# SilverlightningY/dmmt-jpeg-encoder

Hardware: AMD Instinct MI355X
Metric: Mpixel/s encoded (4K PPM, q=90) (higher is better)
Workload: dtype f32; 1 GPU; 3840x2160 synthetic RGB u8, 4:4:4, IJG quality 90, 1 frame(s) per step per GPU, pixels in HBM -> JPEG files in HBM, inputs rotating over 12 distinct slots (285 MiB: streamed from HBM); width=3840, height=2160, subsampling=P444, quality=90, parallelism=independent frames x1, lanes=4, input_slots=12

## Files before the change

### dmmt-jpeg-encoder_amd/csrc/entropy.hip

```cpp
#include <hip/hip_runtime.h>
#include <stdint.h>

#include "device_common.hpp"
#include "jpeg_common.hpp"
#include "kernels.hpp"
#include "slot_copy.hpp"

namespace dmmt {

#ifdef DMMT_PHASE_TRACE
static __device__ unsigned long long g_trace[64];
#endif

static_assert(kChunkBlocks == 256 || kChunkBlocks == 512, "one thread per block, one workgroup per chunk");
constexpr int kEmitThreads = kChunkBlocks;
constexpr int kEmitWaves = kEmitThreads / 64;
#ifndef DMMT_EMIT_OCC
#define DMMT_EMIT_OCC 7
#endif
constexpr int kEmitOcc = kChunkBlocks == 256 ? DMMT_EMIT_OCC : 3;

constexpr int kEmitWords = 4 * kChunkBlocks;
constexpr int kStuffPass = 4096;
#ifndef DMMT_EMIT_BRANCHFREE
#define DMMT_EMIT_BRANCHFREE 1
#endif
#ifndef DMMT_TAIL_DMA
#define DMMT_TAIL_DMA 1
#endif
#ifndef DMMT_TAIL_NSEG1
#define DMMT_TAIL_NSEG1 1
#endif
#ifndef DMMT_EMIT_PRIO_ALWAYS
#define DMMT_EMIT_PRIO_ALWAYS 0
#endif
#ifndef DMMT_EMIT_PRIO
#define DMMT_EMIT_PRIO 1
#endif

struct ChunkSpan {
    long long el0;
    int nb;
    int seg;
    bool seg_first, seg_last;
};

__device__ __forceinline__ ChunkSpan chunk_span(const Geom& g, int c) {
    ChunkSpan r;
    r.seg = min(c / g.cps, g.nseg - 1);
    const int j = c - r.seg * g.cps;
    const long long sb = (long long)r.seg * g.seg_blocks;
    const long long se = min(sb + g.seg_blocks, g.bpf);
    r.el0 = sb + (long long)j * kChunkBlocks;
    r.nb = (int)min((long long)kChunkBlocks, se - r.el0);
    r.seg_first = j == 0;
    r.seg_last = r.el0 + r.nb == se;
    return r;
}

__device__ __forceinline__ bool joined_tail(const Geom& g, int c) {
    return c == g.nch - 1 && g.more_after && g.restart_interval == 0;
}

__device__ __forceinline__ int mod_small(int x, int d, uint32_t inv16) {
    return x - (int)__umul24((uint32_t)d, __umul24((uint32_t)x, inv16) >> 16);
}

struct BlockCoef {
    uint32_t w[32];
};

__device__ __forceinline__ void load_block(const int16_t* __restrict__ p, BlockCoef& b) {
    const uint4* q = reinterpret_cast<const uint4*>(p);
#pragma unroll
    for (int i = 0; i < 8; ++i) {
        const uint4 v = q[i];
        b.w[4 * i] = v.x;
        b.w[4 * i + 1] = v.y;
        b.w[4 * i + 2] = v.z;
        b.w[4 * i + 3] = v.w;
    }
}

__device__ __forceinline__ int coef_at(const BlockCoef& b, int k) {
    return (k & 1) ? ((int)b.w[k >> 1] >> 16) : (int)(int16_t)(b.w[k >> 1] & 0xFFFFu);
}

__device__ __forceinline__ void zigzag_in_registers(BlockCoef& b) {
    uint32_t z[32];
#pragma unroll
    for (int j = 0; j < 32; ++j) {
        const int i0 = coef_pos(2 * j), i1 = coef_pos(2 * j + 1);
        const uint32_t lo = (b.w[i0 >> 1] >> (16 * (i0 & 1))) & 0xFFFFu;
        const uint32_t hi = (b.w[i1 >> 1] >> (16 * (i1 & 1))) & 0xFFFFu;
        z[j] = lo | (hi << 16);
    }
#pragma unroll
    for (int j = 0; j < 32; ++j) b.w[j] = z[j];
}

template <typename Sink>
__device__ __forceinline__ void walk_block(const BlockCoef& b, int dcd, const uint2* __restrict__ dctab,
                                           const uint2* __restrict__ actab, Sink& sink, int kmax = 63) {
    {
        const int cat = category_of(dcd);
        const uint2 e = dctab[cat];
        sink(e.x | extra_bits(dcd, cat), (int)e.y);
    }
    const uint2 z = actab[0xF0];
    int l16 = 16;
#pragma unroll
    for (int k = 1; k < 64; ++k) {
        if (k > kmax) continue;
        const int v = coef_at(b, k);
        if (v != 0) {
            const int r16 = 16 * k - l16;
            for (int r = r16 >> 8; r > 0; --r) sink(z.x, (int)z.y);
            const int cat = category_fast(v);
            const uint2 e = actab[(r16 & 0xF0) | cat];
            sink(e.x | extra_bits(v, cat), (int)e.y);
            l16 = 16 * k + 16;
        }
    }
    if (l16 < 16 * 64 || kmax < 63) {
        const uint2 e = actab[0];
        sink(e.x, (int)e.y);
    }
}

struct CountSink {
    uint32_t n = 0;
    __device__ __forceinline__ void operator()(uint32_t, int len) { n += (uint32_t)len; }
};

struct WindowSink {
    uint32_t* img;
    int lo, n;
    unsigned long long acc;
    int nacc;
    int w;
    bool first;
    __device__ __forceinline__ void put(uint32_t word, bool shared) {
        const int i = w - lo;
        if ((unsigned)i < (unsigned)n) {
            if (shared)
                atomicOr(&img[i], word);
            else
                img[i] = word;
        }
    }
    __device__ __forceinline__ void operator()(uint32_t val, int len) {
        acc = (acc << len) | val;
        nacc += len;
        if (nacc >= 32) {
            nacc -= 32;
            put((uint32_t)(acc >> nacc), first);
            first = false;
            ++w;
        }
    }
    __device__ __forceinline__ void finish() {
        if (nacc > 0) put((uint32_t)(acc << (32 - nacc)), true);
    }
};


struct SlotSink {
    uint32_t* slot;
    unsigned long long acc;
    int nacc;
    int wi;
#if DMMT_EMIT_BRANCHFREE
    __device__ __forceinline__ void operator()(uint32_t val, int len) {
        acc = (acc << len) | val;
        nacc += len;
        const int full = nacc >> 5;
        nacc &= 31;
        slot[min(wi, kSlotWords - 1) * kEmitThreads] = (uint32_t)(acc >> nacc);
        wi += full;
    }
#else
    __device__ __forceinline__ void operator()(uint32_t val, int len) {
        acc = (acc << len) | val;
        nacc += len;
        if (nacc >= 32) {
            nacc -= 32;
            slot[min(wi, kSlotWords - 1) * kEmitThreads] = (uint32_t)(acc >> nacc);
            ++wi;
        }
    }
#endif
    __device__ __forceinline__ uint32_t finish() {
        if (nacc > 0 && wi < kSlotWords) slot[wi * kEmitThreads] = (uint32_t)(acc << (32 - nacc));
        return (uint32_t)wi * 32u + (uint32_t)nacc;
    }
};


__device__ __forceinline__ uint32_t bits16_at(uint32_t a, uint32_t b, int p) {
    const unsigned long long x = ((unsigned long long)a << 32) | b;
    return (uint32_t)(x >> (48 - (p & 31))) & 0xFFFFu;
}

struct NoMark {
    template <typename I>
    __device__ void operator()(I) const {}
};
template <typename Mark = NoMark>
__device__ __forceinline__ void fused_offsets(const uint32_t* __restrict__ cbits, const uint32_t* __restrict__ cff,
                              const unsigned long long* __restrict__ cff8, uint8_t* sFF8,
                              const uint32_t* __restrict__ cedge, const Geom& g, unsigned long long* __restrict__ bit0,
                              unsigned long long* __restrict__ outo, unsigned long long* __restrict__ total,
                              unsigned long long* sWaveV, int* sWaveF, Mark mark = Mark());
static_assert(kArriveWords == kArriveFrameWords, "the host sizes the counters");

__global__ __launch_bounds__(kEmitThreads, kEmitOcc) void k_emit(const int16_t* coef, const int16_t* __restrict__ dcdiff,
                                              const uint8_t* __restrict__ lastnz,
                                              const uint32_t* __restrict__ code_tab, Geom g,
                                              uint32_t* __restrict__ stage, uint32_t* __restrict__ chunk_bits,
                                              uint32_t* __restrict__ chunk_ff, uint32_t* __restrict__ chunk_edge,
                                              uint32_t* __restrict__ ac_hist, uint32_t* __restrict__ dc_hist,
                                              int fuse, uint32_t* __restrict__ arrive,
                                              unsigned long long* __restrict__ chunk_bit0,
                                              unsigned long long* __restrict__ chunk_out,
                                              unsigned long long* __restrict__ total_out,
                                              unsigned long long* __restrict__ chunk_ff8, int prio) {
    __shared__ uint2 sTab[2 * 256 + 2 * 16];
    __shared__ uint32_t sW[kEmitWords + 2];
    __shared__ __attribute__((aligned(16))) uint32_t sSlot[kSlotWords * kEmitThreads];
    __shared__ uint32_t sWave[kEmitWaves];
    __shared__ uint32_t sFF[8];
    __shared__ uint32_t sEdge[3];
    __shared__ uint32_t sBin[65];
    __shared__ unsigned long long sOffV[kEmitWaves + 1];
    __shared__ int sOffF[kEmitWaves];
    __shared__ uint32_t sLast;
    using OrderT = std::conditional_t<(kEmitThreads > 256), uint16_t, uint8_t>;
    uint32_t* const sBits = sW;
    OrderT* const sOrder = reinterpret_cast<OrderT*>(sW + kEmitThreads);
    uint8_t* const sKey = reinterpret_cast<uint8_t*>(sW + kEmitThreads + kEmitThreads * (int)sizeof(OrderT) / 4);
    DMMT_TRACE_START;
    const int tid = threadIdx.x, lane = lane_id(), wave = tid >> 6;
    const int frame = blockIdx.y;
    const unsigned chunk = blockIdx.x;
    const ChunkSpan span = chunk_span(g, (int)chunk);
    const long long el0 = span.el0;
    const int nb = span.nb;
    const long long e = (long long)frame * g.bpf + el0 + tid;
    const size_t cid = (size_t)frame * g.nch + chunk;
    const int r0 = (int)((uint32_t)el0 % (uint32_t)g.bpm);
    const uint32_t inv16 = (65536u + (uint32_t)g.bpm - 1u) / (uint32_t)g.bpm;
    const bool valid = tid < nb;
    const uint32_t* ct = code_tab + (size_t)frame * 1024;
    const int tt = tid & 255;
    const uint32_t tac0 = ct[256 + tt], tac1 = ct[768 + tt];
    const uint32_t tdc = ct[((tt & 31) < 16 ? 0 : 512 - 16) + (tt & 31)];
    const uint32_t lz = lastnz[valid ? e : (long long)frame * g.bpf + el0];
    if (tid < 256) {
        const int c = tid & 15;
        sTab[tid] = make_uint2((tac0 & 0xFFFFu) << c, (tac0 >> 16) + c);
        sTab[256 + tid] = make_uint2((tac1 & 0xFFFFu) << c, (tac1 >> 16) + c);
    }
    if (tid < 32) sTab[512 + tid] = make_uint2((tdc & 0xFFFFu) << (tid & 15), (tdc >> 16) + (tid & 15));
    if (chunk == 0) {
        for (int i = tid; i < kHistReps * 512; i += kEmitThreads) ac_hist[(size_t)frame * kHistReps * 512 + i] = 0u;
        for (int i = tid; i < kHistReps * 32; i += kEmitThreads) dc_hist[(size_t)frame * kHistReps * 32 + i] = 0u;
    }
    if (tid < 8) sFF[tid] = 0u;
    if (tid < 3) sEdge[tid] = 0u;
    if (tid < 65) sBin[tid] = 0u;
    const int key = valid ? (int)lz : 64;
    __syncthreads();
    const uint32_t rank = atomicAdd(&sBin[key], 1u);
    __syncthreads();
// ... 442 lines not shown
        bool f = false;
        unsigned long long v = 0;
#pragma unroll
        for (int i = 0; i < KP; ++i)
            if (c0 + i < c1) seg_combine(f, v, first[i], nbits[i] + (c0 + i == 0 ? (uint32_t)g.bit_phase : 0u));
        unsigned long long run = block_segscan_1024(f, v, sWave, sWaveF);
        unsigned long long b0[KP], ob[KP], mine = 0;
#pragma unroll
        for (int i = 0; i < KP; ++i) {
            const int c = c0 + i;
            b0[i] = ob[i] = 0;
            if (c >= c1) continue;
            if (first[i]) run = c == 0 ? (unsigned long long)g.bit_phase : 0ull;
            b0[i] = run;
            const unsigned long long e = run + nbits[i];
            unsigned long long o = ((e + 7) >> 3) - ((run + 7) >> 3);
            const int rsd = (8 - (int)(run & 7)) & 7;
            uint32_t ffc = 0;
#pragma unroll
            for (int r = 0; r < 8; ++r) ffc = r == rsd ? ffr[i][r] : ffc;
            o += ffc;
            if ((e & 7) && (e & ~7ull) >= run) {
                const uint32_t byte = boundary_byte((int)(e & 7), edge[i] & 0xFFFFu, hasn[i], nnext[i], enext[i] >> 16);
                o += byte == 0xFFu ? 1u : 0u;
            }
            if (segl[i] && (c != nch - 1 || (g.more_after && g.restart_interval > 0))) o += 2;
            ob[i] = o;
            mine += o;
            run = e;
        }
        unsigned long long tot = 0;
        unsigned long long orun = block_scan_1024(mine, sWave, &tot);
#pragma unroll
        for (int i = 0; i < KP; ++i) {
            const int c = c0 + i;
            if (c >= c1) continue;
            bit0[c] = b0[i];
            outo[c] = orun;
            orun += ob[i];
        }
        if (tid == 0) total_out[frame] = tot;
        return;
    }

    bool f = false;
    unsigned long long v = 0;
    for (int c = c0; c < c1; ++c)
        seg_combine(f, v, chunk_span(g, c).seg_first, cbits[c] + (c == 0 ? (unsigned long long)g.bit_phase : 0ull));
    unsigned long long run = block_segscan_1024(f, v, sWave, sWaveF);
    unsigned long long mine = 0;
    for (int c = c0; c < c1; ++c) {
        if (chunk_span(g, c).seg_first) run = c == 0 ? (unsigned long long)g.bit_phase : 0ull;
        bit0[c] = run;
        mine += chunk_out_bytes(cff, cbits, cedge, g, c, run);
        run += cbits[c];
    }
    unsigned long long tot = 0;
    unsigned long long orun = block_scan_1024(mine, sWave, &tot);
    for (int c = c0; c < c1; ++c) {
        outo[c] = orun;
        orun += chunk_out_bytes(cff, cbits, cedge, g, c, bit0[c]);
    }
    if (tid == 0) total_out[frame] = tot;
}

__global__ __launch_bounds__(256, 8) void k_stuffwrite(const uint32_t* __restrict__ stage,
                                                    const uint32_t* __restrict__ chunk_bits,
                                                    const uint32_t* __restrict__ chunk_edge,
                                                    const unsigned long long* __restrict__ chunk_bit0,
                                                    const unsigned long long* __restrict__ chunk_out,
                                                    const unsigned long long* __restrict__ total_out,
                                                    const uint32_t* __restrict__ hdr_len, Geom g,
                                                    uint8_t* __restrict__ out, size_t out_stride,
                                                    uint32_t* __restrict__ out_len, int* __restrict__ status) {
    __shared__ uint32_t sWave[4];
    __shared__ __attribute__((aligned(16))) uint8_t sOut[2 * kStuffPass + 16];
    const int tid = threadIdx.x, lane = lane_id(), wave = tid >> 6;
    const int frame = blockIdx.y;
    const int c = blockIdx.x;
    const size_t cid = (size_t)frame * g.nch + c;
    const bool last = c == g.nch - 1;
    const size_t cidn = last ? cid : cid + 1;
    const uint32_t hdr = hdr_len[frame];
    const unsigned long long tot = total_out[frame];
    const unsigned long long b0 = chunk_bit0[cid];
    const uint32_t n = chunk_bits[cid], edge = chunk_edge[cid];
    const uint32_t n_next = chunk_bits[cidn], edge_next = chunk_edge[cidn];
    const unsigned long long cout = chunk_out[cid], cout_next = chunk_out[cidn];
    const uint32_t* slot = stage + cid * (size_t)kChunkWordsCap;
    uint32_t wv0[5];
    {
        const uint4 q = *reinterpret_cast<const uint4*>(slot + 4 * tid);
        wv0[0] = q.x, wv0[1] = q.y, wv0[2] = q.z, wv0[3] = q.w;
        wv0[4] = slot[4 * tid + 4];
    }
    asm volatile("" ::"s"(hdr), "s"(tot), "s"(b0), "s"(n), "s"(edge), "s"(n_next), "s"(edge_next), "s"(cout),
                 "s"(cout_next), "v"(wv0[0]), "v"(wv0[1]), "v"(wv0[2]), "v"(wv0[3]), "v"(wv0[4]));
    const unsigned long long end = (unsigned long long)hdr + tot;
    if (end + 2 > out_stride) {
        if (c == 0 && tid == 0) {
            out_len[frame] = 0;
            raise_status(status, 16);
        }
        return;
    }
    {
        const unsigned long long cend = last ? tot : cout_next;
        const unsigned long long sbytes = ((unsigned long long)n + 7) / 8 + 1;
        if (n > (uint32_t)kChunkWordsCap * 32u || cout > cend || cend > tot ||
            (unsigned long long)hdr + cout + 2 * sbytes > out_stride) {
            if (tid == 0) {
                out_len[frame] = 0;
                raise_status(status, 16);
            }
            return;
        }
    }
    const ChunkSpan sp = chunk_span(g, c);
    uint8_t* const base = out + (size_t)frame * out_stride + hdr;
    if (tid == 0) {
        if (last && !g.more_after) {
            base[tot] = 0xFF;
            base[tot + 1] = 0xD9;
            out_len[frame] = (uint32_t)(end + 2);
        } else if (sp.seg_last && g.restart_interval > 0) {
            const unsigned long long at = (last ? tot : cout_next) - 2;
            base[at] = 0xFF;
            base[at + 1] = (uint8_t)(0xD0 + ((g.seg_base + sp.seg) & 7));
            if (last) out_len[frame] = (uint32_t)end;
        } else if (last) {
            out_len[frame] = (uint32_t)end;
        }
    }
    const unsigned long long e = b0 + n;
    const unsigned long long kbeg = (b0 + 7) >> 3, kend = (e + 7) >> 3;
    if (kend <= kbeg) return;
    const unsigned long long nbytes = kend - kbeg;
    const bool shared_tail = (e & 7) != 0;
    uint32_t tail = 0;
    if (shared_tail) {
        const bool jt = joined_tail(g, c);
        const bool has_next = !sp.seg_last || jt;
        tail = boundary_byte((int)(e & 7), edge & 0xFFFFu, has_next,
                             jt ? (uint32_t)g.next_bits : (has_next ? n_next : 0u),
                             jt ? g.next16 : (has_next ? edge_next >> 16 : 0u));
    }
    const unsigned off = (unsigned)(8 * kbeg - b0);
    uint8_t* o = base + cout;
    for (unsigned long long pos = 0; pos < nbytes; pos += kStuffPass) {
        const uint32_t delta = (uint32_t)(reinterpret_cast<uintptr_t>(o) & 15u);
        const unsigned long long kb = pos + 16u * (unsigned)tid;
        const int nvalid = kb < nbytes ? (int)min(16ull, nbytes - kb) : 0;
        uint32_t x[4] = {0u, 0u, 0u, 0u};
        uint32_t cnt = 0;
        if (nvalid) {
            const unsigned long long p = off + 8 * kb;
            const size_t wi = (size_t)(p >> 5);
            const int sh = (int)(p & 31);
            uint32_t wv[5];
#pragma unroll
            for (int i = 0; i < 5; ++i) wv[i] = pos ? slot[wi + i] : wv0[i];
#pragma unroll
            for (int i = 0; i < 4; ++i) x[i] = sh ? (wv[i] << sh) | (wv[i + 1] >> (32 - sh)) : wv[i];
            if (shared_tail && nbytes - 1 - kb < 16) {
                const int j = (int)(nbytes - 1 - kb), sft = 24 - 8 * (j & 3);
                x[j >> 2] = (x[j >> 2] & ~(0xFFu << sft)) | (tail << sft);
            }
#pragma unroll
            for (int i = 0; i < 4; ++i) {
                const int nv = min(max(nvalid - 4 * i, 0), 4);
                const uint32_t vmask = nv ? 0x80808080u & (0xFFFFFFFFu << (32 - 8 * nv)) : 0u;
                const uint32_t t = ~x[i];
                const uint32_t nonzero = (((t & 0x7F7F7F7Fu) + 0x7F7F7F7Fu) | t) & 0x80808080u;
                cnt += (uint32_t)__popc(~nonzero & vmask);
            }
        }
        const uint32_t incl = wave_incl_scan_full_u32(cnt);
        if (lane == 63) sWave[wave] = incl;
        __syncthreads();
        uint32_t pre = incl - cnt;
        for (int q = 0; q < wave; ++q) pre += sWave[q];
        const uint32_t ffs = sWave[0] + sWave[1] + sWave[2] + sWave[3];
        if (nvalid) {
            uint32_t dst = delta + (uint32_t)tid * 16u + pre;
#pragma unroll
            for (int j = 0; j < 16; ++j) {
                if (j < nvalid) {
                    const uint32_t b = (x[j >> 2] >> (24 - 8 * (j & 3))) & 0xFFu;
                    sOut[dst++] = (uint8_t)b;
                    if (b == 0xFFu) sOut[dst++] = 0x00;
                }
            }
        }
        __syncthreads();
        const unsigned long long in_pass = nbytes - pos < (unsigned long long)kStuffPass ? nbytes - pos : kStuffPass;
        const uint32_t len = (uint32_t)in_pass + ffs;
        const uint32_t send = delta + len;
        uint8_t* const oa = o - delta;
        for (uint32_t sb = 16u * (uint32_t)tid; sb < send; sb += 16u * 256u) {
            if (sb >= delta && sb + 16u <= send) {
                *reinterpret_cast<uint4*>(oa + sb) = *reinterpret_cast<const uint4*>(sOut + sb);
            } else {
                for (uint32_t i = max(sb, delta); i < min(sb + 16u, send); ++i) oa[i] = sOut[i];
            }
        }
        o += len;
        __syncthreads();
    }
}

bool offsets_fusable(const Geom& g) { return g.nch <= kFusedOffsetsMaxChunks; }

hipError_t launch_emit(int n_frames, const Geom& g, const Work& w, bool fuse_offsets, hipStream_t st, bool prio) {
    const int fuse = fuse_offsets && offsets_fusable(g) ? 1 : 0;
    hipLaunchKernelGGL(k_emit, dim3(g.nch, n_frames), dim3(kEmitThreads), 0, st, (const int16_t*)w.coef,
                       (const int16_t*)w.dcdiff, (const uint8_t*)w.lastnz, (const uint32_t*)w.code_tab, g, w.stage, w.chunk_bits, w.chunk_ff,
                       w.chunk_edge, w.ac_hist, w.dc_hist, fuse, w.arrive, w.chunk_bit0, w.chunk_out, w.total_out,
                       w.chunk_ff8, prio || DMMT_EMIT_PRIO_ALWAYS ? 1 : 0);
    return hipGetLastError();
}

hipError_t launch_offsets(int n_frames, const Geom& g, const Work& w, hipStream_t st) {
    hipLaunchKernelGGL(k_offsets, dim3(n_frames), dim3(1024), 0, st, (const uint32_t*)w.chunk_bits,
                       (const uint32_t*)w.chunk_ff, (const uint32_t*)w.chunk_edge, g, w.chunk_bit0, w.chunk_out,
                       w.total_out);
    return hipGetLastError();
}

hipError_t launch_stuffwrite(int n_frames, const Geom& g, const Work& w, uint8_t* out, size_t out_stride,
                             uint32_t* out_len, hipStream_t st) {
    hipLaunchKernelGGL(k_stuffwrite, dim3(g.nch, n_frames), dim3(256), 0, st, (const uint32_t*)w.stage,
                       (const uint32_t*)w.chunk_bits, (const uint32_t*)w.chunk_edge,
                       (const unsigned long long*)w.chunk_bit0, (const unsigned long long*)w.chunk_out,
                       (const unsigned long long*)w.total_out, (const uint32_t*)w.hdr_len, g, out, out_stride,
                       out_len, w.status);
    return hipGetLastError();
}

}

#ifdef DMMT_PHASE_TRACE
extern "C" int dmmt_debug_trace_entropy(unsigned long long* out64) {
    if (hipMemcpyFromSymbol(out64, HIP_SYMBOL(dmmt::g_trace), 64 * 8) != hipSuccess) return -1;
    unsigned long long z[64] = {0};
    return hipMemcpyToSymbol(HIP_SYMBOL(dmmt::g_trace), z, sizeof z) == hipSuccess ? 0 : -1;
}
#endif
```

### dmmt-jpeg-encoder_amd/csrc/kernels.hip

```cpp

#include <hip/hip_runtime.h>
#include <stdint.h>
#include <stdlib.h>

#include <type_traits>

#include "dct_quant.hpp"
#include "device_common.hpp"
#include "front_launch.hpp"
#include "jpeg_common.hpp"
#include "kernels.hpp"
#include "surface_load.hpp"
#include "wave_merge.hpp"

namespace dmmt {

#ifdef DMMT_PHASE_TRACE
static __device__ unsigned long long g_trace[64];
#endif

__constant__ uint8_t c_zigzag[64] = {0,  1,  8,  16, 9,  2,  3,  10, 17, 24, 32, 25, 18, 11, 4,  5,
                                     12, 19, 26, 33, 40, 48, 41, 34, 27, 20, 13, 6,  7,  14, 21, 28,
                                     35, 42, 49, 56, 57, 50, 43, 36, 29, 22, 15, 23, 30, 37, 44, 51,
                                     58, 59, 52, 45, 38, 31, 39, 46, 53, 60, 61, 54, 47, 55, 62, 63};
__constant__ uint8_t c_inv_zigzag[64] = {0,  1,  5,  6,  14, 15, 27, 28, 2,  4,  7,  13, 16, 26, 29, 42,
                                         3,  8,  12, 17, 25, 30, 41, 43, 9,  11, 18, 24, 31, 40, 44, 53,
                                         10, 19, 23, 32, 39, 45, 52, 54, 20, 22, 33, 38, 46, 51, 55, 60,
                                         21, 34, 37, 47, 50, 56, 59, 61, 35, 36, 48, 49, 57, 58, 62, 63};

__device__ __forceinline__ void rgb_to_ycbcr(float r, float g, float b, float& y, float& cb, float& cr) {
    const float k128 = 128.0f / 255.0f;
    y = (((r * 0.299f + g * 0.587f) + b * 0.114f) - k128) * 255.0f;
    cb = ((r * -0.1687f + g * -0.3312f) + b * 0.5f) * 255.0f;
    cr = ((r * 0.5f + g * -0.4186f) + b * -0.0813f) * 255.0f;
}


template <typename Sample, int ROWS>
struct RawTile {
    static constexpr int RB = 256 * 3 * (int)sizeof(Sample);
    static constexpr int RC = RB / 16 + 1;
    static constexpr int RS = RC * 16;
    static constexpr int NCHUNK = ROWS * RC;
    static constexpr int NQ = (NCHUNK + 255) / 256;
    static constexpr int BYTES = NCHUNK * 16;

    __device__ static __forceinline__ long long row_start(const Geom& g, int x0, int py) {
        return ((long long)py * g.width + x0) * 3 * (long long)sizeof(Sample);
    }
    __device__ static __forceinline__ int misalign(const uint8_t* fbase, long long start) {
        return (int)(((uintptr_t)fbase + (uintptr_t)start) & 15u);
    }

    __device__ static __forceinline__ int misalign32(const uint8_t* fbase, const Geom& g, int x0, int py) {
        return (int)(((uint32_t)(uintptr_t)fbase + (uint32_t)(py * g.width + x0) * (uint32_t)(3 * sizeof(Sample))) & 15u);
    }

    __device__ static __forceinline__ void load(const uint8_t* __restrict__ fbase, long long fbytes, const Geom& g,
                                                int x0, int y0, int tid, uint4 (&v)[NQ]) {
        const long long last = row_start(g, x0, y0 + ROWS - 1);
        if (x0 + 256 <= g.width && y0 + ROWS <= g.height && row_start(g, x0, y0) >= 16 && last + RB + 16 <= fbytes) {
            const uint8_t* tb = fbase + row_start(g, x0, y0);
            const uint32_t rowpitch = (uint32_t)g.width * (uint32_t)(3 * sizeof(Sample));
#pragma unroll
            for (int i = 0; i < NQ; ++i) {
                const int q = tid + 256 * i;
                const int row = q / RC, j = q - (q / RC) * RC;
                const uint8_t* r = tb + (size_t)((uint32_t)row * rowpitch);
                const uint8_t* a = r - ((uint32_t)(uintptr_t)r & 15u) + 16u * (uint32_t)j;
                v[i] = q < NCHUNK ? ld16_nt(a) : make_uint4(0u, 0u, 0u, 0u);
            }
            return;
        }
        const long long rowbytes = (long long)min(256, g.width - x0) * 3 * (long long)sizeof(Sample);
#pragma unroll
        for (int i = 0; i < NQ; ++i) {
            v[i] = make_uint4(0u, 0u, 0u, 0u);
            const int q = tid + 256 * i;
            const int row = q / RC, j = q - (q / RC) * RC;
            const int py = y0 + row;
            if (q >= NCHUNK || py >= g.height) continue;
            const long long start = row_start(g, x0, py);
            const long long c = start - misalign(fbase, start) + 16LL * j;
            if (c >= start + rowbytes) continue;
            if (c >= 0 && c + 16 <= fbytes) {
                v[i] = ld16_nt(fbase + c);
            } else {
                uint32_t w[4] = {0u, 0u, 0u, 0u};
                for (int k = 0; k < 16; ++k)
                    if (c + k >= 0 && c + k < fbytes) w[k >> 2] |= (uint32_t)fbase[c + k] << (8 * (k & 3));
                v[i] = make_uint4(w[0], w[1], w[2], w[3]);
            }
            const long long keep = start + rowbytes - c;
            if (keep < 16) {
                uint32_t w[4] = {v[i].x, v[i].y, v[i].z, v[i].w};
#pragma unroll
                for (int k = 0; k < 4; ++k) {
                    const long long n = keep - 4 * k;
                    w[k] &= n >= 4 ? 0xFFFFFFFFu : (n <= 0 ? 0u : (1u << (8 * n)) - 1u);
                }
                v[i] = make_uint4(w[0], w[1], w[2], w[3]);
            }
        }
    }

    __device__ static __forceinline__ void stage(uint8_t* sRaw, int tid, const uint4 (&v)[NQ]) {
#pragma unroll
        for (int i = 0; i < NQ; ++i) {
            const int q = tid + 256 * i;
            if (q < NCHUNK) reinterpret_cast<uint4*>(sRaw)[q] = v[i];
        }
    }
};

enum { LAY_TIGHT = 0, LAY_RGB = 1, LAY_RGBX = 2, LAY_PLANAR = 3 };
template <int LAY>
struct SurfLayout {
    static constexpr int NPL = LAY == LAY_PLANAR ? 3 : 1;
    static constexpr int SPP = LAY == LAY_RGBX ? 4 : (LAY == LAY_PLANAR ? 1 : 3);
};
struct SurfMem {
    const uint8_t* base;
    __device__ __forceinline__ void load16(long long off, uint32_t (&w)[4]) const {
        const uint4 v = ld16_nt(base + off);
        w[0] = v.x, w[1] = v.y, w[2] = v.z, w[3] = v.w;
    }
    __device__ __forceinline__ uint32_t load1(long long off) const { return base[off]; }
};
template <typename Sample, int ROWS, int LAY>
struct SurfTile {
    static constexpr int NPL = SurfLayout<LAY>::NPL;
    static constexpr int BPP = SurfLayout<LAY>::SPP * (int)sizeof(Sample);
    static constexpr int RB = 256 * BPP;
    static constexpr int RC = RB / 16 + 1;
    static constexpr int RS = RC * 16;
    static constexpr int NCHUNK = ROWS * NPL * RC;
    static constexpr int NQ = (NCHUNK + 255) / 256;
    static constexpr int BYTES = NCHUNK * 16;

    struct Planes {
        const uint8_t *p0, *p1, *p2;
    };
    __device__ static __forceinline__ Planes planes(const SurfArgs& sa, size_t foff) {
        return Planes{sa.plane[0] + foff, sa.plane[NPL == 1 ? 0 : 1] + foff, sa.plane[NPL == 1 ? 0 : 2] + foff};
    }
    __device__ static __forceinline__ const uint8_t* plane(const Planes& pl, int p) {
        return NPL == 1 || p == 0 ? pl.p0 : (p == 1 ? pl.p1 : pl.p2);
    }
    __device__ static __forceinline__ int misalign32(const uint8_t* pbase, const SurfArgs& sa, int x0, int py) {
        return surf_misalign32((uint32_t)(uintptr_t)pbase, (uint32_t)sa.pitch, BPP, x0, py);
    }

    __device__ static __forceinline__ void load(const SurfArgs& sa, size_t foff, const Geom& g, int x0, int y0, int tid,
                                                uint4 (&v)[NQ]) {
        const Planes pl = planes(sa, foff);
        const long long first = surf_row_start(sa.pitch, BPP, x0, y0);
        if (x0 + 256 <= g.width && y0 + ROWS <= g.height &&
            surf_interior(first, surf_row_start(sa.pitch, BPP, x0, y0 + ROWS - 1), RB, sa.span)) {
#pragma unroll
            for (int i = 0; i < NQ; ++i) {
                const int q = tid + 256 * i;
                const int tr = q / RC, j = q - (q / RC) * RC;
                const int row = tr / NPL, p = tr - (tr / NPL) * NPL;
                const uint8_t* pb = plane(pl, p);
                const long long c = surf_interior_chunk((uint32_t)(uintptr_t)pb, first + (long long)row * sa.pitch, j);
                v[i] = q < NCHUNK ? ld16_nt(pb + c) : make_uint4(0u, 0u, 0u, 0u);
            }
            return;
        }
        const long long rowbytes = surf_row_bytes(g.width, BPP, x0);
#pragma unroll
        for (int i = 0; i < NQ; ++i) {
            v[i] = make_uint4(0u, 0u, 0u, 0u);
            const int q = tid + 256 * i;
            const int tr = q / RC, j = q - (q / RC) * RC;
            const int row = tr / NPL, p = tr - (tr / NPL) * NPL;
            const int py = y0 + row;
            if (q >= NCHUNK || py >= g.height) continue;
            const SurfMem m{plane(pl, p)};
            uint32_t w[4];
            surf_load_chunk(m, surf_row_start(sa.pitch, BPP, x0, py), misalign32(m.base, sa, x0, py), rowbytes, sa.span,
                            j, w);
            v[i] = make_uint4(w[0], w[1], w[2], w[3]);
        }
    }

    __device__ static __forceinline__ void stage(uint8_t* sRaw, int tid, const uint4 (&v)[NQ]) {
// ... 25 lines not shown
    constexpr int SB = (int)sizeof(Sample);
    constexpr int NPL = SurfLayout<LAY>::NPL;
    constexpr int SPP = SurfLayout<LAY>::SPP;
    constexpr int PXB = 8 * SPP * SB;
    constexpr int PXW = PXB / 4;
    constexpr int NCJ = NB * 8;
    constexpr int JPT = (NCJ + 255) / 256;
    using Raw = std::conditional_t<LAY == LAY_TIGHT, RawTile<Sample, ROWS>, SurfTile<Sample, ROWS, LAY>>;

    __shared__ __attribute__((aligned(16))) float sT[NB * BS + 4];
    __shared__ __attribute__((aligned(16))) uint8_t sRaw[Raw::BYTES];
    __shared__ float sLut[256];
    __shared__ float sQ[128];
    __shared__ float sRQ[128];

    DMMT_TRACE_START;
    const int tid = threadIdx.x;
    const int frame = blockIdx.y;
    const uint8_t* fbase = nullptr;
    long long fbytes = 0;
    size_t foff = 0;
    if constexpr (LAY == LAY_TIGHT) {
        fbase = reinterpret_cast<const uint8_t*>(rgb + (size_t)frame * frame_stride);
        fbytes = (long long)g.width * g.height * 3 * SB;
    } else {
        foff = (size_t)frame * frame_stride;
    }
    if (tid < 128) sQ[tid] = qtab[tid];
    if (tid < 128) sRQ[tid] = SB == 4 ? 1.0f / qtab[tid] : c_arai_scale[(tid >> 3) & 7] * (1.0f / qtab[tid]);
    if (SB == 1) sLut[tid] = norm_lut[tid];
    const int col = tid & 7;

    const int tiles_per_row = (g.mcux + TM - 1) / TM;
    const int ntiles = tiles_per_row * g.mcuy;
    int bad = 0;
    const bool check_range = SB != 4 && g.maxval < (SB == 1 ? 255 : 65535);

    uint4 raw[Raw::NQ];
    auto load_tile = [&](int tx0, int ty0) {
        if constexpr (LAY == LAY_TIGHT)
            Raw::load(fbase, fbytes, g, tx0, ty0, tid, raw);
        else
            Raw::load(sa, foff, g, tx0, ty0, tid, raw);
    };
    if ((int)blockIdx.x < ntiles) {
        const int my = blockIdx.x / tiles_per_row;
        load_tile((blockIdx.x - my * tiles_per_row) * TM * 8 * HR, my * ROWS);
    }
    for (int tile = blockIdx.x; tile < ntiles; tile += gridDim.x) {
        const int my = tile / tiles_per_row;
        const int mx0 = (tile - my * tiles_per_row) * TM;
        const int x0 = mx0 * 8 * HR;
        const int y0 = my * ROWS;

        Raw::stage(sRaw, tid, raw);
        __syncthreads();
        {
            const int nt = tile + gridDim.x;
            if (nt < ntiles) {
                const int ny = nt / tiles_per_row;
                load_tile((nt - ny * tiles_per_row) * TM * 8 * HR, ny * ROWS);
            }
        }

        auto phase_a = [&](auto range_check) {
            constexpr bool CHECK = decltype(range_check)::value;
            const int h = tid % SP, job = tid / SP;
            const int c = job % CB, r = job / CB;
            const int lx0 = c * 8 * HR + 8 * h;
            uint32_t pw[VR * NPL][SB == 4 ? 1 : PXW];
            const float* fsrc[VR * NPL];
#pragma unroll
            for (int dy = 0; dy < VR; ++dy) {
#pragma unroll
                for (int p = 0; p < NPL; ++p) {
                    const int ly = r * VR + dy;
                    int mis;
                    if constexpr (LAY == LAY_TIGHT)
                        mis = Raw::misalign32(fbase, g, x0, y0 + ly);
                    else
                        mis = Raw::misalign32(sa.plane[p] + foff, sa, x0, y0 + ly);
                    const uint8_t* src = sRaw + (ly * NPL + p) * Raw::RS + mis + lx0 * SPP * SB;
                    fsrc[dy * NPL + p] = reinterpret_cast<const float*>(src);
                    if constexpr (SB == 4) {
                        pw[dy * NPL + p][0] = 0u;
                    } else if ((mis & 7) == 0) {
#pragma unroll
                        for (int k = 0; k < PXW / 2; ++k) {
                            const uint2 u = reinterpret_cast<const uint2*>(src)[k];
                            pw[dy * NPL + p][2 * k] = u.x;
                            pw[dy * NPL + p][2 * k + 1] = u.y;
                        }
                    } else {
#pragma unroll
                        for (int k = 0; k < PXW; ++k)
                            pw[dy * NPL + p][k] = (uint32_t)src[4 * k] | ((uint32_t)src[4 * k + 1] << 8) |
                                                  ((uint32_t)src[4 * k + 2] << 16) | ((uint32_t)src[4 * k + 3] << 24);
                    }
                }
            }
            float yv[VR][8];
            float cbv[8], crv[8];
            uint32_t smax = 0;
#pragma unroll
            for (int k = 0; k < NCS; ++k) {
                float cbs = 0.0f, crs = 0.0f;
#pragma unroll
                for (int dx = 0; dx < HR; ++dx) {
#pragma unroll
                    for (int dy = 0; dy < VR; ++dy) {
                        const int jx = k * HR + dx;
                        float rr, gg, bb;
                        if constexpr (SB == 4) {
                            if constexpr (LAY == LAY_PLANAR) {
                                rr = fsrc[dy * NPL][jx];
                                gg = fsrc[dy * NPL + 1][jx];
                                bb = fsrc[dy * NPL + 2][jx];
                            } else {
                                rr = fsrc[dy][jx * SPP];
                                gg = fsrc[dy][jx * SPP + 1];
                                bb = fsrc[dy][jx * SPP + 2];
                                if constexpr (LAY != LAY_TIGHT) {
                                    const float s0 = rr;
                                    rr = sa.bgr ? bb : rr;
                                    bb = sa.bgr ? s0 : bb;
                                }
                            }
                        } else {
                            uint32_t sv[3];
#pragma unroll
                            for (int ch = 0; ch < 3; ++ch) {
                                const int si = LAY == LAY_PLANAR ? jx : jx * SPP + ch;
                                const uint32_t* rw = pw[LAY == LAY_PLANAR ? dy * NPL + ch : dy];
                                sv[ch] = SB == 1 ? (rw[si >> 2] >> (8 * (si & 3))) & 0xFFu
                                                 : (rw[si >> 1] >> (16 * (si & 1))) & 0xFFFFu;
                            }
                            if constexpr (LAY == LAY_RGB || LAY == LAY_RGBX) {
                                const uint32_t s0 = sv[0];
                                sv[0] = sa.bgr ? sv[2] : sv[0];
                                sv[2] = sa.bgr ? s0 : sv[2];
                            }
                            if constexpr (CHECK) smax = max(smax, max(sv[0], max(sv[1], sv[2])));
                            if (SB == 1) {
                                rr = sLut[sv[0]];
                                gg = sLut[sv[1]];
                                bb = sLut[sv[2]];
                            } else {
                                rr = norm_lut[sv[0]];
                                gg = norm_lut[sv[1]];
                                bb = norm_lut[sv[2]];
                            }
                        }
                        float y, cb, cr;
                        rgb_to_ycbcr(rr, gg, bb, y, cb, cr);
                        yv[dy][jx] = y;
                        if (dx == 0 && dy == 0) {
                            cbs = cb;
                            crs = cr;
                        } else {
                            cbs = cbs + cb;
                            crs = crs + cr;
                        }
                    }
                }
                if (HR * VR > 1) {
                    cbs = cbs / (float)(HR * VR);
                    crs = crs / (float)(HR * VR);
                }
                cbv[k] = cbs;
                crv[k] = crs;
            }
            if constexpr (CHECK) bad |= (int)(smax > (uint32_t)g.maxval);
#pragma unroll
            for (int dy = 0; dy < VR; ++dy) {
                const int ly = r * VR + dy;
                arai8(yv[dy]);
                float4* o = reinterpret_cast<float4*>(sT + blk_base((ly >> 3) * 32 + c * HR + h) + (ly & 7) * 8);
                o[0] = make_float4(yv[dy][0], yv[dy][1], yv[dy][2], yv[dy][3]);
                o[1] = make_float4(yv[dy][4], yv[dy][5], yv[dy][6], yv[dy][7]);
            }
            if constexpr (SP == 1) {
                arai8(cbv);
                arai8(crv);
                float4* ob = reinterpret_cast<float4*>(sT + blk_base(NYB + c) + r * 8);
                ob[0] = make_float4(cbv[0], cbv[1], cbv[2], cbv[3]);
                ob[1] = make_float4(cbv[4], cbv[5], cbv[6], cbv[7]);
                float4* orr = reinterpret_cast<float4*>(sT + blk_base(NYB + CB + c) + r * 8);
                orr[0] = make_float4(crv[0], crv[1], crv[2], crv[3]);
                orr[1] = make_float4(crv[4], crv[5], crv[6], crv[7]);
            } else {
                float fr[8];
#pragma unroll
                for (int k = 0; k < 4; ++k) {
                    const float send = h ? cbv[k] : crv[k];
                    const float recv = __int_as_float(
                        __builtin_amdgcn_update_dpp(0, __float_as_int(send), 0xB1, 0xF, 0xF, false));
                    fr[k] = h ? recv : cbv[k];
                    fr[4 + k] = h ? crv[k] : recv;
                }
                arai8(fr);
                float4* oc = reinterpret_cast<float4*>(sT + blk_base(NYB + (h ? CB : 0) + c) + r * 8);
                oc[0] = make_float4(fr[0], fr[1], fr[2], fr[3]);
                oc[1] = make_float4(fr[4], fr[5], fr[6], fr[7]);
            }
        };
        if (tid < NJ) {
            if (check_range)
                phase_a(std::integral_constant<bool, true>{});
            else
                phase_a(std::integral_constant<bool, false>{});
        }
        __syncthreads();
        DMMT_TRACE(0);

        const int nvalid = min(TM, g.mcux - mx0) * BPM;
        const long long e0 = (long long)frame * g.bpf + ((long long)my * g.mcux + mx0) * BPM;
        int16_t* const cbase = coef + e0 * 64;
        static_assert(NCJ % 256 == 0, "JPT column jobs for every thread");
#pragma unroll
        for (int jj = 0; jj < JPT; ++jj) {
            const int blk = (tid + 256 * jj) >> 3;
            int x[8];
            {
                const float* q = sQ + (blk < NYB ? 0 : 64) + col;
                const float* rq = sRQ + (blk < NYB ? 0 : 64) + col;
                float v[8];
                const float* tb = sT + blk_base(blk) + col;
#pragma unroll
                for (int i = 0; i < 8; ++i) v[i] = tb[i * 8];
                if constexpr (SB == 4) {
                    arai8(v);
                    quantize_col8(v, q, rq, x);
                } else {
                    arai8_unscaled(v);
                    quantize_col8_scaled(v, q, rq, g.maxval == 0, x);
                }
            }
            int el;
            if (blk < NYB) {
                const int by = blk / 32, bx = blk % 32;
                el = (bx / HR) * BPM + by * HR + (bx % HR);
            } else if (blk < NYB + CB) {
                el = (blk - NYB) * BPM + NLUMA;
            } else {
                el = (blk - NYB - CB) * BPM + NLUMA + 1;
            }
            const bool valid = el < nvalid;
            if (valid) {
                uint32_t pk[4];
#pragma unroll
                for (int i = 0; i < 4; ++i) pk[i] = __builtin_amdgcn_perm((uint32_t)x[2 * i + 1], (uint32_t)x[2 * i], 0x05040100u);
                *reinterpret_cast<uint4*>(cbase + (el * 64 + 8 * col)) = make_uint4(pk[0], pk[1], pk[2], pk[3]);
            }
        }
        DMMT_TRACE(2);
    }

    if (bad) raise_status(status, bad);
    DMMT_TRACE(5);
    DMMT_TRACE_FLUSH(0, 0);
}

template <int HR, int VR, typename Sample, int WPE>
__global__ __launch_bounds__(256, WPE) void k_front(const Sample* __restrict__ rgb, size_t frame_stride, Geom g,
                                               const float* __restrict__ norm_lut,
                                               const float* __restrict__ qtab,
                                               int16_t* __restrict__ coef, int* __restrict__ status) {
    front_body<HR, VR, Sample, LAY_TIGHT>(rgb, frame_stride, SurfArgs{}, g, norm_lut, qtab, coef, status);
}

template <int HR, int VR, typename Sample, int LAY, int WPE>
__global__ __launch_bounds__(256, WPE) void k_front_surf(SurfArgs sa, size_t frame_stride, Geom g,
                                                    const float* __restrict__ norm_lut,
                                                    const float* __restrict__ qtab, int16_t* __restrict__ coef,
                                                    int* __restrict__ status) {
    front_body<HR, VR, Sample, LAY>(nullptr, frame_stride, sa, g, norm_lut, qtab, coef, status);
}

struct HistCoef {
    uint32_t w[32];
};

constexpr int kTailSmallWords = 4 + 4 * 16;
__device__ __forceinline__ void tables_tail(uint8_t* lds, const uint32_t* ac_hist, const uint32_t* dc_hist, int frame,
                                            const Geom& g, uint32_t* __restrict__ code_tab, uint8_t* __restrict__ out,
                                            size_t out_stride, uint32_t* __restrict__ hdr_len,
                                            const uint8_t* __restrict__ qtab_u8, int bits_per_channel,
                                            int* __restrict__ status, int* sCnt, int* sBits);
constexpr int kHistCopies = 4, kHistCopyWords = 545;
constexpr int kTailLdsBytes = 7072;

template <bool CHECK, bool FUSE>
__global__ __launch_bounds__(256) __attribute__((amdgpu_waves_per_eu(8, 8))) void k_hist(const int16_t* __restrict__ coef, int16_t* __restrict__ dcdiff,
                                              uint8_t* __restrict__ lastnz, Geom g,
                                              uint32_t* __restrict__ ac_hist ,
                                              uint32_t* __restrict__ dc_hist ,
                                              int* __restrict__ status, uint32_t* __restrict__ arrive,
                                              uint32_t* __restrict__ code_tab, uint8_t* __restrict__ out,
                                              size_t out_stride, uint32_t* __restrict__ hdr_len,
                                              const uint8_t* __restrict__ qtab_u8, int bits_per_channel) {
    constexpr int NC = kHistCopies, HS = kHistCopyWords;
    constexpr int kWords = FUSE && kTailLdsBytes / 4 > NC * HS ? kTailLdsBytes / 4 : NC * HS;
    __shared__ __attribute__((aligned(16))) uint32_t sH[kWords];
    __shared__ int sSmall[FUSE ? kTailSmallWords : 1];
    __shared__ uint32_t sLastWg;
    const int tid = threadIdx.x;
    const int frame = blockIdx.y;
// ... 904 lines not shown
```

Measured before the change: 191,500 Mpixel/s.

## Restructure AC walk, branch-free byte stuffing, simplified copy-out, FMA color convert

The AC Huffman walk now tests nonzero coefficients directly on packed words in groups of four and exits early past kmax. It also guards the ZRL run loop with a wave-uniform ballot so most waves skip it. Byte stuffing scatters bytes to positions derived from popcounts of the 0xFF mask and writes the zero bytes in a separate sparse loop, replacing the serial per-byte loop. The copy-out loop handles only full 16-byte vectors, with edge bytes written by 32 dedicated threads, and the color conversion uses explicit FMAs for the 0.5 terms when SB!=4, which can change rounding.

Measured after the change: 194,300 Mpixel/s, median of 6. 1.5% higher.

```diff
diff --git a/dmmt-jpeg-encoder_amd/csrc/entropy.hip b/dmmt-jpeg-encoder_amd/csrc/entropy.hip
--- a/dmmt-jpeg-encoder_amd/csrc/entropy.hip
+++ b/dmmt-jpeg-encoder_amd/csrc/entropy.hip
@@ -108,18 +108,29 @@
         sink(e.x | extra_bits(dcd, cat), (int)e.y);
     }
     const uint2 z = actab[0xF0];
+    uint32_t m_run = 0xF0u, m_low = 0xFFFFu, m_zrl = 255u;
+    asm volatile("" : "+s"(m_run), "+s"(m_low), "+s"(m_zrl));
     int l16 = 16;
 #pragma unroll
-    for (int k = 1; k < 64; ++k) {
-        if (k > kmax) continue;
-        const int v = coef_at(b, k);
-        if (v != 0) {
-            const int r16 = 16 * k - l16;
-            for (int r = r16 >> 8; r > 0; --r) sink(z.x, (int)z.y);
-            const int cat = category_fast(v);
-            const uint2 e = actab[(r16 & 0xF0) | cat];
-            sink(e.x | extra_bits(v, cat), (int)e.y);
-            l16 = 16 * k + 16;
+    for (int k0 = 0; k0 < 64; k0 += 4) {
+        if (k0 != 0 && k0 > kmax) break;
+#pragma unroll
+        for (int k = k0 ? k0 : 1; k < k0 + 4; ++k) {
+            const uint32_t w = b.w[k >> 1];
+            if ((k & 1) ? w > m_low : (w << 16) != 0u) {
+                const int v = coef_at(b, k);
+                const int r16 = 16 * k - l16;
+                if (k >= 17 && __builtin_amdgcn_ballot_w64((uint32_t)r16 > m_zrl) != 0) {
+                    int r = r16 >> 8;
+                    asm volatile("" : "+v"(r));
+#pragma unroll 1
+                    for (; r > 0; --r) sink(z.x, (int)z.y);
+                }
+                const int cat = category_fast(v);
+                const uint2 e = actab[(r16 & (int)m_run) | cat];
+                sink(e.x | extra_bits(v, cat), (int)e.y);
+                l16 = 16 * k + 16;
+            }
         }
     }
     if (l16 < 16 * 64 || kmax < 63) {
@@ -868,6 +879,7 @@
         const unsigned long long kb = pos + 16u * (unsigned)tid;
         const int nvalid = kb < nbytes ? (int)min(16ull, nbytes - kb) : 0;
         uint32_t x[4] = {0u, 0u, 0u, 0u};
+        uint32_t ffm[4] = {0u, 0u, 0u, 0u};
         uint32_t cnt = 0;
         if (nvalid) {
             const unsigned long long p = off + 8 * kb;
@@ -888,7 +900,8 @@
                 const uint32_t vmask = nv ? 0x80808080u & (0xFFFFFFFFu << (32 - 8 * nv)) : 0u;
                 const uint32_t t = ~x[i];
                 const uint32_t nonzero = (((t & 0x7F7F7F7Fu) + 0x7F7F7F7Fu) | t) & 0x80808080u;
-                cnt += (uint32_t)__popc(~nonzero & vmask);
+                ffm[i] = ~nonzero & vmask;
+                cnt += (uint32_t)__popc(ffm[i]);
             }
         }
         const uint32_t incl = wave_incl_scan_full_u32(cnt);
@@ -898,13 +911,27 @@
         for (int q = 0; q < wave; ++q) pre += sWave[q];
         const uint32_t ffs = sWave[0] + sWave[1] + sWave[2] + sWave[3];
         if (nvalid) {
-            uint32_t dst = delta + (uint32_t)tid * 16u + pre;
-#pragma unroll
-            for (int j = 0; j < 16; ++j) {
-                if (j < nvalid) {
-                    const uint32_t b = (x[j >> 2] >> (24 - 8 * (j & 3))) & 0xFFu;
-                    sOut[dst++] = (uint8_t)b;
-                    if (b == 0xFFu) sOut[dst++] = 0x00;
+            const uint32_t dst = delta + (uint32_t)tid * 16u + pre;
+            uint32_t a = dst;
+#pragma unroll
+            for (int i = 0; i < 4; ++i) {
+                const uint32_t w = x[i], f = ffm[i];
+                sOut[a + 4 * i] = (uint8_t)(w >> 24);
+                sOut[a + (uint32_t)__popc(f & 0x80000000u) + 4 * i + 1] = (uint8_t)(w >> 16);
+                sOut[a + (uint32_t)__popc(f & 0x80800000u) + 4 * i + 2] = (uint8_t)(w >> 8);
+                sOut[a + (uint32_t)__popc(f & 0x80808000u) + 4 * i + 3] = (uint8_t)w;
+                a += (uint32_t)__popc(f);
+            }
+            if (cnt) {
+                uint32_t m = 0;
+#pragma unroll
+                for (int i = 0; i < 4; ++i)
+                    m |= ((((ffm[i] >> 7) * 0x08040201u) >> 24) & 0xFu) << (4 * i);
+                uint32_t z = dst + 1;
+                while (m) {
+                    sOut[z + (uint32_t)__builtin_ctz(m)] = 0x00;
+                    ++z;
+                    m &= m - 1u;
                 }
             }
         }
@@ -913,12 +940,14 @@
         const uint32_t len = (uint32_t)in_pass + ffs;
         const uint32_t send = delta + len;
         uint8_t* const oa = o - delta;
-        for (uint32_t sb = 16u * (uint32_t)tid; sb < send; sb += 16u * 256u) {
-            if (sb >= delta && sb + 16u <= send) {
-                *reinterpret_cast<uint4*>(oa + sb) = *reinterpret_cast<const uint4*>(sOut + sb);
-            } else {
-                for (uint32_t i = max(sb, delta); i < min(sb + 16u, send); ++i) oa[i] = sOut[i];
-            }
+        for (uint32_t sb = 16u * (uint32_t)tid; sb + 16u <= send; sb += 16u * 256u) {
+            if (sb >= delta) *reinterpret_cast<uint4*>(oa + sb) = *reinterpret_cast<const uint4*>(sOut + sb);
+        }
+        if (tid < 32) {
+            const uint32_t sbt = send & ~15u;
+            const uint32_t i = tid < 16 ? (uint32_t)tid : sbt + (uint32_t)tid - 16u;
+            const bool mine = tid < 16 ? i >= delta && (delta > 0u || send < 16u) : sbt > 0u;
+            if (mine && i < send) oa[i] = sOut[i];
         }
         o += len;
         __syncthreads();
diff --git a/dmmt-jpeg-encoder_amd/csrc/kernels.hip b/dmmt-jpeg-encoder_amd/csrc/kernels.hip
--- a/dmmt-jpeg-encoder_amd/csrc/kernels.hip
+++ b/dmmt-jpeg-encoder_amd/csrc/kernels.hip
@@ -28,11 +28,17 @@
                                          10, 19, 23, 32, 39, 45, 52, 54, 20, 22, 33, 38, 46, 51, 55, 60,
                                          21, 34, 37, 47, 50, 56, 59, 61, 35, 36, 48, 49, 57, 58, 62, 63};
 
+template <bool HALF_FMA>
 __device__ __forceinline__ void rgb_to_ycbcr(float r, float g, float b, float& y, float& cb, float& cr) {
     const float k128 = 128.0f / 255.0f;
     y = (((r * 0.299f + g * 0.587f) + b * 0.114f) - k128) * 255.0f;
-    cb = ((r * -0.1687f + g * -0.3312f) + b * 0.5f) * 255.0f;
-    cr = ((r * 0.5f + g * -0.4186f) + b * -0.0813f) * 255.0f;
+    if constexpr (HALF_FMA) {
+        cb = __builtin_fmaf(b, 0.5f, r * -0.1687f + g * -0.3312f) * 255.0f;
+        cr = (__builtin_fmaf(r, 0.5f, g * -0.4186f) + b * -0.0813f) * 255.0f;
+    } else {
+        cb = ((r * -0.1687f + g * -0.3312f) + b * 0.5f) * 255.0f;
+        cr = ((r * 0.5f + g * -0.4186f) + b * -0.0813f) * 255.0f;
+    }
 }
 
 
@@ -364,7 +370,7 @@
                             }
                         }
                         float y, cb, cr;
-                        rgb_to_ycbcr(rr, gg, bb, y, cb, cr);
+                        rgb_to_ycbcr<SB != 4>(rr, gg, bb, y, cb, cr);
                         yv[dy][jx] = y;
                         if (dx == 0 && dy == 0) {
                             cbs = cb;
```
